# nv-tlabs/LION

Hardware: AMD Instinct MI355X
Metric: shapes/sec @1000-step DDIM, Bx2048pts (higher is better)
Workload: dtype f32 (operands of the 3x3x3 voxel convolutions and of the long 1x1 convolutions cut into fp16 hi/lo pairs on the 16-bi...

## Files before the change

### include/lion_hip.h

```cpp
#ifndef LION_HIP_H_
#define LION_HIP_H_

#include <stddef.h>
#include <stdint.h>

#ifdef __cplusplus
extern "C" {
#endif

typedef void *lionStream_t;

#define LION_OK 0
#define LION_EINVAL (-1)
#define LION_EUNSUPPORTED (-2)
#define LION_EWORKSPACE (-3)

int lion_abi_version(void);

size_t lion_avg_voxelize_workspace_bytes(int B, int C, int N, int r);
int lion_avg_voxelize_forward(const float *feat, const int32_t *coords, int B, int C, int N,
                              int r, float *out, int32_t *ind, int32_t *cnt, void *ws,
                              size_t ws_bytes, lionStream_t stream);

int lion_voxelize_points_forward(const float *feat, const float *coords, int B, int C, int N,
// ... 133 lines not shown
int lion_conv3d_stat_tiles(int r, int Cout, int B, int sparse);
int lion_conv3d_k3_fused_forward(const float *x, const float *wp, const float *bias, int B, int Cin,
                                 int Cout, int r, const float *pro_a, const float *pro_b, const float *pro_bias,
                                 const float *tconst, float *y, float *stats, int32_t *occ, lionStream_t stream);
size_t lion_conv3d_occupancy_ints(int r, int Cout, int B);
int lion_conv3d_const_response(const float *wsum, const float *bias2, const float *bias1, const float *pro_a,
                               const float *pro_b, int B, int Cin, int Cout, float *tconst, lionStream_t stream);
int lion_conv3d_tile_occupancy(const int32_t *cnt, int B, int r, int Cout, int32_t *occ_m1, int32_t *occ_m2,
                               lionStream_t stream);
int lion_conv3d_tile_occupancy_aware(const int32_t *cnt, int B, int r, int Cout, int32_t *occ_m1, int32_t *occ_m2,
                                     int consumer_aware, lionStream_t stream);
int lion_groupnorm_fold(const float *stats, int B, int C, int T, int G, int voxels, const float *gamma,
                        const float *beta, const float *fac, const float *gbias, int ld_fg, float eps,
                        float *A, float *Bs, float *chmean, lionStream_t stream);
size_t lion_conv3d_split_packed_halfs(int Cout, int Cin);
int lion_conv3d_split_pack_weights(const float *w, int Cout, int Cin, uint16_t *wp, lionStream_t stream);
int lion_conv3d_split_stat_tiles(int r, int Cout);
int lion_conv3d_k3_split_forward(const float *x, const uint16_t *wp, const float *bias, int B, int Cin, int Cout,
                                 int r, const float *pro_a, const float *pro_b, const float *pro_bias,
                                 const float *tconst, float *y, float *stats, int32_t *occ, lionStream_t stream);
int lion_conv3d_k3_half_forward(const float *x, const uint16_t *wp, const float *bias, int B, int Cin, int Cout,
                                int r, const float *pro_a, const float *pro_b, const float *pro_bias,
                                const float *tconst, float *y, float *stats, int32_t *occ, lionStream_t stream);
size_t lion_skinny_packed_floats(int Cout, int Cin);
int lion_skinny_pack_weights(const float *w, int Cout, int Cin, float *wp, lionStream_t stream);
int lion_skinny_splits(int Cin, int Cout);
int lion_skinny_gemm(const float *pin, int ks_in, const float *bias_in, int act_in, const float *addT,
                     const float *wp, int nb, int Cin, int Cout, float *pout, lionStream_t stream);
int lion_skinny_finish(const float *A, int ks_a, const float *bias_a, const float *Bp, int ks_b, const float *resid,
                       int nb, int C, int mode, float *y, lionStream_t stream);
int lion_skinny_gemm_se_finish(const float *pin, int ks_in, const float *bias_in, int act_in, const float *wp, int nb, int Cin,
                               int Cout, const float *A, int ks_a, const float *bias_a, const float *resid, float *y,
                               lionStream_t stream);
int lion_to_channel_major(const float *a, int lda, int Ca, float *oa, const float *b, int ldb, int Cb, float *ob, int B,
                          lionStream_t stream);
int lion_from_channel_major(const float *x, int B, int C, float *y, lionStream_t stream);
int lion_groupnorm_fold_se(const float *stats, int B, int C, int T, int G, int voxels, const float *gamma,
                           const float *beta, const float *fac, const float *gbias, int ld_fg, float eps, const float *w1,
                           const float *w2, int H, float *A, float *Bs, lionStream_t stream);
int lion_se_gate(const float *chmean, const float *w1, const float *w2, int B, int C, int H, float *A,
                 float *Bs, lionStream_t stream);
int lion_trilinear_devoxelize_affine_forward(const float *coords, const float *feat, const float *scale,
                                             const float *shift, int B, int C, int N, int r, float *out,
                                             lionStream_t stream);
size_t lion_devoxelize_plan_bytes(int B, int N, int r);
int lion_trilinear_devoxelize_plan(const float *coords, int B, int N, int r, void *plan, size_t plan_bytes,
                                   lionStream_t stream);
int lion_trilinear_devoxelize_planned_forward(const void *plan, size_t plan_bytes, const float *coords, const float *feat,
                                              const float *scale, const float *shift, int B, int C, int N, int r,
                                              float *out, lionStream_t stream);

int lion_row_stats(const float *x, int rows, int L, float *stats, lionStream_t stream);
size_t lion_pwconv_packed_floats(int Cout, int Cin);
int lion_pwconv_pack_weights(const float *w, int Cout, int Cin, float *wp, lionStream_t stream);
int lion_pwconv_stat_tiles(int Cout, int Cin, int L);
int lion_pwconv_forward(const float *x, const float *wp, const float *bias, int B, int Cin, int Cout, int L,
                        const float *pro_a, const float *pro_b, float *y, float *stats, lionStream_t stream);
int lion_pwconv_forward_max(const float *x, const float *wp, const float *bias, int B, int Cin, int Cout, int L,
                            const float *pro_a, const float *pro_b, const float *out_a, const float *out_b,
                            float *stats, float *ymax, lionStream_t stream);
size_t lion_pwconv_split_packed_halfs(int Cout, int Cin);
int lion_pwconv_split_pack_weights(const float *w, int Cout, int Cin, uint16_t *wp, lionStream_t stream);
int lion_pwconv_split_pack_weights_t(const float *w, int Cout, int Cin, const uint16_t *wp, uint16_t *wpt, lionStream_t stream);
int lion_pwconv_split_stat_tiles(int Cout, int Cin, int L);
int lion_pwconv_split_forward(const float *x, const uint16_t *wp, const float *bias, int B, int Cin, int Cout, int L,
                              const float *pro_a, const float *pro_b, float *y, float *stats, lionStream_t stream);
int lion_pwconv_grouped_forward(const float *coords, const float *centers, const float *feat, const int32_t *idx,
                                const float *wp, const float *bias, int B, int C, int N, int M, int U, int Cout, float *y,
                                float *stats, lionStream_t stream);
int lion_pwconv_split_grouped_forward(const float *coords, const float *centers, const float *feat, const int32_t *idx,
                                      const uint16_t *wp, const float *bias, int B, int C, int N, int M, int U, int Cout,
                                      float *y, float *stats, lionStream_t stream);
int lion_internal_pwconv_walk(const float *x, const float *wp, const float *bias, int B, int Cin, int Cout, int L,
                              const float *pro_a, const float *pro_b, const float *out_a, const float *out_b,
                              const float *coords, const float *centers, const float *feat, const int32_t *idx, int N, int U,
                              float *y, float *stats, int max_wg, int lds_weights, lionStream_t stream);
int lion_linear_attention_core(const float *qkv, int B, int H, int D, int N, float *out, lionStream_t stream);
int lion_linear_attention_core_backward(const float *qkv, const float *gout, int B, int H, int D, int N, float *gqkv,
                                        lionStream_t stream);
int lion_linear_forward(const float *x, const float *wp, const float *bias, int B, int K, int O, int act, float slope,
                        float *y, lionStream_t stream);
int lion_affine_swish(const float *x, const float *A, const float *Bs, int rows, int L, float *y,
                      lionStream_t stream);
int lion_affine_swish_max(const float *x, const float *A, const float *Bs, int rows, int M, int U,
                          float *y, lionStream_t stream);
int lion_timestep_embedding(const float *t, const float *row, float scale, int B, int half, int D, float *emb,
                            lionStream_t stream);
int lion_affine_swish_add(const float *x, const float *A, const float *Bs, const float *addend, int rows, int L, float *y,
                          lionStream_t stream);

size_t lion_scatter_csr_workspace_bytes(int B, int E, int bins);
int lion_scatter_csr(const float *gy, const int32_t *idx, const float *w, int B, int C, int S, int E, int bins, void *ws,
                     size_t ws_bytes, float *gx, lionStream_t stream);

size_t lion_pwconv_wgrad_workspace_bytes(int B, int Cin, int Cout, int L);
int lion_pwconv_wgrad(const float *x, const float *gy, int B, int Cin, int Cout, int L, void *ws, size_t ws_bytes,
                      float *gw, float *gb, lionStream_t stream);

int lion_gn_train_fold(const float *stats, const float *gw, const float *gb, const float *fac, int fac_stride,
                       const float *bias, int bias_stride, int B, int C, int G, int L, float eps, float *A, float *Bs,
                       float *mean, float *rstd, lionStream_t stream);
int lion_row_stats64(const float *x, int rows, int L, double *stats, lionStream_t stream);
int lion_gn_train_fold64(const double *stats, const float *gw, const float *gb, const float *fac, int fac_stride,
                         const float *bias, int bias_stride, int B, int C, int G, int L, float eps, float *A,
                         float *Bs, float *mean, float *rstd, lionStream_t stream);
int lion_gn_train_bwd_fold(const float *S, const float *mean, const float *rstd, const float *gw, const float *gb,
                           const float *fac, int fac_stride, int B, int C, int G, int L, float *Q, float *R, float *dfac,
                           float *dbias, int d_stride, float *pw, const float *A, const double *xstats, const float *gate,
                           const float *qse, float *Aout, lionStream_t stream);
int lion_gn_train_param_grads(const float *pw, int B, int C, float *dgw, float *dgb, float *dxs, lionStream_t stream);
// ... 71 lines not shown
```

### lion_amd/_lib.py

```python
from __future__ import annotations

import ctypes as C
import os

_HERE = os.path.dirname(os.path.abspath(__file__))
SO_PATH = os.environ.get("LION_HIP_SO") or os.path.join(_HERE, "csrc", "liblion_hip.so")

_vp, _i, _f, _sz = C.c_void_p, C.c_int, C.c_float, C.c_size_t

SIGNATURES = {
    "lion_abi_version": (_i, []),
    "lion_avg_voxelize_workspace_bytes": (_sz, [_i, _i, _i, _i]),
    "lion_avg_voxelize_forward": (_i, [_vp, _vp, _i, _i, _i, _i, _vp, _vp, _vp, _vp, _sz, _vp]),
    "lion_voxelize_points_forward": (_i, [_vp, _vp, _i, _i, _i, _i, _i, _f, _vp, _vp, _vp, _vp,
                                          _vp, _sz, _vp]),
    "lion_voxel_plan_bytes": (_sz, [_i, _i, _i]),
    "lion_voxel_index": (_i, [_vp, _i, _i, _i, _i, _f, _vp, _vp, _vp, _vp, _sz, _vp]),
    "lion_voxel_scatter": (_i, [_vp, _vp, _sz, _i, _i, _i, _i, _vp, _vp]),
    "lion_voxel_scatter_read": (_i, [_vp, _vp, _sz, _i, _i, _i, _i, _vp, _vp, _vp]),
    "lion_avg_voxelize_backward": (_i, [_vp, _vp, _vp, _i, _i, _i, _i, _vp, _vp]),
    "lion_trilinear_devoxelize_forward": (_i, [_vp, _vp, _i, _i, _i, _i, _i, _vp, _vp, _vp, _vp]),
    "lion_trilinear_devoxelize_backward": (_i, [_vp, _vp, _vp, _i, _i, _i, _i, _vp, _vp]),
    "lion_ball_query": (_i, [_vp, _vp, _i, _i, _i, _f, _i, _vp, _vp]),
    "lion_grouping_forward": (_i, [_vp, _vp, _i, _i, _i, _i, _i, _vp, _vp]),
# ... 9 lines not shown
    "lion_chamfer_loss_reduce": (_i, [_vp, _vp, _i, _i, _i, _f, _f, _vp, _vp]),
    "lion_chamfer_loss_backward": (_i, [_vp, _vp, _vp, _vp, _vp, _i, _i, _i, _f, _f, _vp, _vp, _vp]),
    "lion_emd_workspace_bytes": (_sz, [_i, _i, _i]),
    "lion_emd_approxmatch": (_i, [_vp, _vp, _i, _i, _i, _vp, _vp, _sz, _vp]),
    "lion_emd_cost": (_i, [_vp, _vp, _i, _i, _i, _vp, _vp, _sz, _vp]),
    "lion_emd_matchcost": (_i, [_vp, _vp, _vp, _i, _i, _i, _vp, _vp, _sz, _vp]),
    "lion_emd_matchcost_backward": (_i, [_vp, _vp, _vp, _vp, _i, _i, _i, _vp, _vp, _vp]),
    "lion_conv3d_packed_floats": (_sz, [_i, _i]),
    "lion_conv3d_pack_weights": (_i, [_vp, _i, _i, _vp, _vp]),
    "lion_conv3d_k3_forward": (_i, [_vp, _vp, _vp, _i, _i, _i, _i, _vp, _vp]),
    "lion_conv3d_wgrad_workspace_floats": (_sz, [_i, _i, _i, _i]),
    "lion_conv3d_k3_wgrad": (_i, [_vp, _vp, _i, _i, _i, _i, _vp, _vp, _sz, _vp]),
    "lion_conv3d_k3_wgrad_split": (_i, [_vp, _vp, _i, _i, _i, _i, _vp, _vp, _sz, _vp]),
    "lion_conv3d_wgrad_sparse_workspace_floats": (_sz, [_i, _i, _i, _i]),
    "lion_conv3d_k3_wgrad_split_sparse": (_i, [_vp, _vp, _vp, _i, _i, _i, _i, _vp, _vp, _sz, _vp]),
    "lion_conv3d_stat_tiles": (_i, [_i, _i, _i, _i]),
    "lion_conv3d_k3_fused_forward": (_i, [_vp, _vp, _vp, _i, _i, _i, _i, _vp, _vp, _vp, _vp, _vp, _vp, _vp, _vp]),
    "lion_conv3d_const_response": (_i, [_vp, _vp, _vp, _vp, _vp, _i, _i, _i, _vp, _vp]),
    "lion_conv3d_occupancy_ints": (_sz, [_i, _i, _i]),
    "lion_conv3d_tile_occupancy": (_i, [_vp, _i, _i, _i, _vp, _vp, _vp]),
    "lion_conv3d_tile_occupancy_aware": (_i, [_vp, _i, _i, _i, _vp, _vp, _i, _vp]),
    "lion_conv3d_split_packed_halfs": (_sz, [_i, _i]),
    "lion_conv3d_split_pack_weights": (_i, [_vp, _i, _i, _vp, _vp]),
    "lion_conv3d_split_stat_tiles": (_i, [_i, _i]),
    "lion_conv3d_k3_split_forward": (_i, [_vp, _vp, _vp, _i, _i, _i, _i, _vp, _vp, _vp, _vp, _vp, _vp, _vp, _vp]),
    "lion_conv3d_k3_half_forward": (_i, [_vp, _vp, _vp, _i, _i, _i, _i, _vp, _vp, _vp, _vp, _vp, _vp, _vp, _vp]),
    "lion_groupnorm_fold": (_i, [_vp, _i, _i, _i, _i, _i, _vp, _vp, _vp, _vp, _i, _f, _vp, _vp, _vp, _vp]),
    "lion_groupnorm_fold_se": (_i, [_vp, _i, _i, _i, _i, _i, _vp, _vp, _vp, _vp, _i, _f, _vp, _vp, _i, _vp, _vp, _vp]),
    "lion_skinny_packed_floats": (_sz, [_i, _i]),
    "lion_skinny_pack_weights": (_i, [_vp, _i, _i, _vp, _vp]),
    "lion_skinny_splits": (_i, [_i, _i]),
    "lion_skinny_gemm": (_i, [_vp, _i, _vp, _i, _vp, _vp, _i, _i, _i, _vp, _vp]),
    "lion_skinny_gemm_se_finish": (_i, [_vp, _i, _vp, _i, _vp, _i, _i, _i, _vp, _i, _vp, _vp, _vp, _vp]),
    "lion_skinny_finish": (_i, [_vp, _i, _vp, _vp, _i, _vp, _i, _i, _i, _vp, _vp]),
    "lion_to_channel_major": (_i, [_vp, _i, _i, _vp, _vp, _i, _i, _vp, _i, _vp]),
    "lion_from_channel_major": (_i, [_vp, _i, _i, _vp, _vp]),
    "lion_se_gate": (_i, [_vp, _vp, _vp, _i, _i, _i, _vp, _vp, _vp]),
    "lion_trilinear_devoxelize_affine_forward": (_i, [_vp, _vp, _vp, _vp, _i, _i, _i, _i, _vp, _vp]),
    "lion_devoxelize_plan_bytes": (_sz, [_i, _i, _i]),
    "lion_trilinear_devoxelize_plan": (_i, [_vp, _i, _i, _i, _vp, _sz, _vp]),
    "lion_trilinear_devoxelize_planned_forward": (_i, [_vp, _sz, _vp, _vp, _vp, _vp, _i, _i, _i, _i, _vp, _vp]),
    "lion_row_stats": (_i, [_vp, _i, _i, _vp, _vp]),
    "lion_pwconv_packed_floats": (_sz, [_i, _i]),
    "lion_pwconv_pack_weights": (_i, [_vp, _i, _i, _vp, _vp]),
    "lion_pwconv_stat_tiles": (_i, [_i, _i, _i]),
    "lion_pwconv_forward": (_i, [_vp, _vp, _vp, _i, _i, _i, _i, _vp, _vp, _vp, _vp, _vp]),
    "lion_pwconv_forward_max": (_i, [_vp, _vp, _vp, _i, _i, _i, _i, _vp, _vp, _vp, _vp, _vp, _vp, _vp]),
    "lion_pwconv_split_packed_halfs": (_sz, [_i, _i]),
    "lion_pwconv_split_pack_weights": (_i, [_vp, _i, _i, _vp, _vp]),
    "lion_pwconv_split_pack_weights_t": (_i, [_vp, _i, _i, _vp, _vp, _vp]),
    "lion_pwconv_split_stat_tiles": (_i, [_i, _i, _i]),
    "lion_pwconv_split_forward": (_i, [_vp, _vp, _vp, _i, _i, _i, _i, _vp, _vp, _vp, _vp, _vp]),
    "lion_pwconv_grouped_forward": (_i, [_vp, _vp, _vp, _vp, _vp, _vp, _i, _i, _i, _i, _i, _i, _vp, _vp, _vp]),
    "lion_pwconv_split_grouped_forward": (_i, [_vp, _vp, _vp, _vp, _vp, _vp, _i, _i, _i, _i, _i, _i, _vp, _vp, _vp]),
    "lion_internal_pwconv_walk": (_i, [_vp, _vp, _vp, _i, _i, _i, _i, _vp, _vp, _vp, _vp, _vp, _vp, _vp, _vp, _i, _i, _vp, _vp, _i, _i, _vp]),
    "lion_linear_attention_core": (_i, [_vp, _i, _i, _i, _i, _vp, _vp]),
    "lion_linear_attention_core_backward": (_i, [_vp, _vp, _i, _i, _i, _i, _vp, _vp]),
    "lion_linear_forward": (_i, [_vp, _vp, _vp, _i, _i, _i, _i, _f, _vp, _vp]),
    "lion_affine_swish": (_i, [_vp, _vp, _vp, _i, _i, _vp, _vp]),
    "lion_affine_swish_max": (_i, [_vp, _vp, _vp, _i, _i, _i, _vp, _vp]),
    "lion_timestep_embedding": (_i, [_vp, _vp, _f, _i, _i, _i, _vp, _vp]),
    "lion_affine_swish_add": (_i, [_vp, _vp, _vp, _vp, _i, _i, _vp, _vp]),
    "lion_scatter_csr_workspace_bytes": (_sz, [_i, _i, _i]),
    "lion_scatter_csr": (_i, [_vp, _vp, _vp, _i, _i, _i, _i, _i, _vp, _sz, _vp, _vp]),
    "lion_pwconv_wgrad_workspace_bytes": (_sz, [_i, _i, _i, _i]),
    "lion_pwconv_wgrad": (_i, [_vp, _vp, _i, _i, _i, _i, _vp, _sz, _vp, _vp, _vp]),
    "lion_gn_train_fold": (_i, [_vp, _vp, _vp, _vp, _i, _vp, _i, _i, _i, _i, _i, _f, _vp, _vp, _vp, _vp, _vp]),
    "lion_row_stats64": (_i, [_vp, _i, _i, _vp, _vp]),
    "lion_gn_train_fold64": (_i, [_vp, _vp, _vp, _vp, _i, _vp, _i, _i, _i, _i, _i, _f, _vp, _vp, _vp, _vp, _vp]),
    "lion_gn_train_bwd_fold": (_i, [_vp, _vp, _vp, _vp, _vp, _vp, _i, _i, _i, _i, _i, _vp, _vp, _vp, _vp, _i, _vp, _vp, _vp, _vp, _vp,
                                    _vp, _vp]),
    "lion_gn_train_param_grads": (_i, [_vp, _i, _i, _vp, _vp, _vp, _vp]),
    "lion_adam_chunk": (_i, []),
    "lion_adam_row": (_i, []),
    "lion_adam_step": (_i, [_vp, _vp, _vp, _i, _i, _vp, _f, _f, _f, _f, _f, _vp]),
    "lion_grad_sqnorm_partials": (_i, [_vp, _vp, _vp, _i, _vp, _vp]),
    "lion_grad_clip_coef": (_i, [_vp, _i, _f, _vp, _vp]),
    "lion_adam_step_scaled": (_i, [_vp, _vp, _vp, _i, _i, _vp, _f, _f, _f, _f, _f, _vp, _vp]),
    "lion_se_gate_fwd": (_i, [_vp, _vp, _vp, _i, _i, _i, _i, _vp, _vp, _vp, _vp, _vp]),
    "lion_se_gate_bwd": (_i, [_vp, _vp, _vp, _vp, _vp, _vp, _i, _i, _i, _i, _vp, _vp, _vp, _vp, _vp, _vp]),
    "lion_rows_dot2": (_i, [_vp, _vp, _vp, _i, _i, _i, _vp, _vp]),
    "lion_trilinear_devoxelize_backward_affine": (_i, [_vp, _vp, _vp, _vp, _vp, _vp, _vp, _i, _i, _i, _i, _vp, _vp]),
    "lion_gn_se_gate_fwd": (_i, [_vp, _vp, _vp, _vp, _vp, _i, _i, _i, _i, _vp, _vp, _vp, _vp, _vp, _vp]),
    "lion_gn_se_gate_bwd": (_i, [_vp, _vp, _vp, _vp, _vp, _vp, _vp, _vp, _vp, _i, _i, _i, _i, _vp, _vp, _vp, _vp, _vp, _vp, _vp]),
    "lion_affine_act": (_i, [_vp, _vp, _vp, _i, _i, _i, _vp, _vp]),
    "lion_affine_act_bwd_stats": (_i, [_vp, _vp, _vp, _vp, _i, _i, _i, _vp, _vp]),
    "lion_affine_act_bwd_apply": (_i, [_vp, _vp, _vp, _vp, _vp, _vp, _i, _i, _i, _vp, _vp]),
    "lion_affine_act_dropout": (_i, [_vp, _vp, _vp, _i, _i, _i, _vp, _f, _vp, _vp]),
    "lion_affine_act_dropout_bwd_stats": (_i, [_vp, _vp, _vp, _vp, _i, _i, _i, _vp, _f, _vp, _vp]),
# ... 107 lines not shown
```

### lion_amd/csrc/attention.hip

```cpp
#include "common.h"
#include <math.h>

namespace {

typedef float f32x16 __attribute__((ext_vector_type(16)));
constexpr int AD = 32;
constexpr int AT = 64;

__global__ __launch_bounds__(256) void linattn_core_kernel(const float *__restrict__ qkv, int H, int N,
                                                           float *__restrict__ out) {
  __shared__ float pT[AT * 33], vT[AT * 33];
  __shared__ float part[4][1024];
  __shared__ float rmax[AD], rinv[AD];
  const int tid = threadIdx.x, lane = tid & 63, wave = tid >> 6, cl = lane & 31, kh = lane >> 5;
  const int h = blockIdx.x, b = blockIdx.y;
  const size_t bs = (size_t)b * 3 * H * AD * N;
  const float *q = qkv + bs + (size_t)(0 * H + h) * AD * N;
  const float *k = qkv + bs + (size_t)(1 * H + h) * AD * N;
  const float *v = qkv + bs + (size_t)(2 * H + h) * AD * N;

  {
    const int d = tid >> 3, sub = tid & 7;
    const float *kr = k + (size_t)d * N;
    float m = -INFINITY;
// ... 31 lines not shown
    }
    __syncthreads();
  }
#pragma unroll
  for (int i = 0; i < 16; ++i) part[wave][((i & 3) + 8 * (i >> 2) + 4 * kh) * 32 + cl] = acc[i];
  __syncthreads();
  float *ctx = pT;
#pragma unroll
  for (int e = tid; e < 1024; e += 256)
    ctx[(e >> 5) * 33 + (e & 31)] = ((part[0][e] + part[1][e]) + part[2][e]) + part[3][e];
  __syncthreads();

  float av[16];
#pragma unroll
  for (int s = 0; s < 16; ++s) av[s] = ctx[(2 * s + kh) * 33 + cl];
  float *ob = out + ((size_t)b * H + h) * AD * N;
  for (int c0 = wave * 32; c0 < N; c0 += 128) {
    const int n = c0 + cl;
    const bool ok = n < N;
    const int nc = ok ? n : N - 1;
    float bv[16];
#pragma unroll
    for (int s = 0; s < 16; ++s) bv[s] = q[(size_t)(2 * s + kh) * N + nc];
    f32x16 o;
#pragma unroll
    for (int i = 0; i < 16; ++i) o[i] = 0.f;
#pragma unroll
    for (int s = 0; s < 16; ++s) o = __builtin_amdgcn_mfma_f32_32x32x2f32(av[s], ok ? bv[s] : 0.f, o, 0, 0, 0);
    if (ok) {
#pragma unroll
      for (int i = 0; i < 16; ++i) ob[(size_t)((i & 3) + 8 * (i >> 2) + 4 * kh) * N + n] = o[i];
    }
  }
}

__global__ __launch_bounds__(256) void linattn_core_bwd_kernel(const float *__restrict__ qkv, const float *__restrict__ gout,
                                                               int H, int N, float *__restrict__ gqkv) {
  __shared__ float pT[AT * 33], vT[AT * 33], qT[AT * 33], gT[AT * 33];
  __shared__ float part[4][1024];
  __shared__ float ctxs[AD * 33], gctxs[AD * 33];
  __shared__ float rmax[AD], rinv[AD], dots[AD];
  const int tid = threadIdx.x, lane = tid & 63, wave = tid >> 6, cl = lane & 31, kh = lane >> 5;
  const int h = blockIdx.x, b = blockIdx.y;
  const size_t bs = (size_t)b * 3 * H * AD * N;
  const float *q = qkv + bs + (size_t)(0 * H + h) * AD * N;
  const float *k = qkv + bs + (size_t)(1 * H + h) * AD * N;
  const float *v = qkv + bs + (size_t)(2 * H + h) * AD * N;
  const float *g = gout + ((size_t)b * H + h) * AD * N;
  float *gq = gqkv + bs + (size_t)(0 * H + h) * AD * N;
  float *gk = gqkv + bs + (size_t)(1 * H + h) * AD * N;
  float *gv = gqkv + bs + (size_t)(2 * H + h) * AD * N;

  {
    const int d = tid >> 3, sub = tid & 7;
    const float *kr = k + (size_t)d * N;
    float m = -INFINITY;
    for (int n = sub; n < N; n += 8) { const float t = kr[n]; m = t > m ? t : m; }
    for (int s = 1; s < 8; s <<= 1) { const float o = __shfl_xor(m, s, 64); m = o > m ? o : m; }
    float sum = 0.f;
    for (int n = sub; n < N; n += 8) sum += expf(kr[n] - m);
    for (int s = 1; s < 8; s <<= 1) sum += __shfl_xor(sum, s, 64);
    if (sub == 0) { rmax[d] = m; rinv[d] = 1.0f / sum; }
  }
  __syncthreads();

  f32x16 acc, gacc;
// ... 63 lines not shown
      bg[s] = ok ? g[(size_t)r_ * N + nc] : 0.f;
      bv[s] = ok ? v[(size_t)r_ * N + nc] : 0.f;
      bp[s] = ok ? expf(k[(size_t)r_ * N + nc] - rmax[r_]) * rinv[r_] : 0.f;
    }
    f32x16 oq, op, ov;
#pragma unroll
    for (int i = 0; i < 16; ++i) oq[i] = op[i] = ov[i] = 0.f;
#pragma unroll
    for (int s = 0; s < 16; ++s) {
      oq = __builtin_amdgcn_mfma_f32_32x32x2f32(aq[s], bg[s], oq, 0, 0, 0);
      op = __builtin_amdgcn_mfma_f32_32x32x2f32(ap[s], bv[s], op, 0, 0, 0);
      ov = __builtin_amdgcn_mfma_f32_32x32x2f32(av[s], bp[s], ov, 0, 0, 0);
    }
    if (ok) {
#pragma unroll
      for (int i = 0; i < 16; ++i) {
        const int row = (i & 3) + 8 * (i >> 2) + 4 * kh;
        gq[(size_t)row * N + n] = oq[i];
        gv[(size_t)row * N + n] = ov[i];
        const float pr = expf(k[(size_t)row * N + n] - rmax[row]) * rinv[row];
        gk[(size_t)row * N + n] = pr * (op[i] - dots[row]);
      }
    }
  }
}

}

extern "C" {

int lion_linear_attention_core(const float *qkv, int B, int H, int D, int N, float *out, lionStream_t stream) {
  if (!qkv || !out || B <= 0 || H <= 0 || N <= 0) return LION_EINVAL;
  if (D != AD) return LION_EUNSUPPORTED;
  return lion_launch<linattn_core_kernel>(dim3(H, B), 256, 0, static_cast<hipStream_t>(stream), qkv, H, N, out);
}

int lion_linear_attention_core_backward(const float *qkv, const float *gout, int B, int H, int D, int N, float *gqkv,
                                        lionStream_t stream) {
  if (!qkv || !gout || !gqkv || B <= 0 || H <= 0 || N <= 0) return LION_EINVAL;
  if (D != AD) return LION_EUNSUPPORTED;
  return lion_launch<linattn_core_bwd_kernel>(dim3(H, B), 256, 0, static_cast<hipStream_t>(stream), qkv, gout, H, N,
                                              gqkv);
}

}
```

### lion_amd/csrc/skinny.hip

```cpp
#include "common.h"

namespace {

typedef float f32x16 __attribute__((ext_vector_type(16)));

typedef float v4f __attribute__((ext_vector_type(4)));
__device__ __forceinline__ float4 ld_stream(const float4 *p) {
  const v4f v = __builtin_nontemporal_load(reinterpret_cast<const v4f *>(p));
  return make_float4(v.x, v.y, v.z, v.w);
}
__device__ __forceinline__ float relu_keep_nan(float v) { return !(v <= 0.f) ? v : 0.f; }

template <bool FIN>
__global__ __launch_bounds__(1024) void skinny_gemm_kernel(const float *__restrict__ pin, int ks_in,
                                                           const float *__restrict__ bias_in, int act_in,
                                                           const float *__restrict__ addT,
                                                           const float *__restrict__ wp, int Cin, int Cout,
                                                           float *__restrict__ pout, const float *__restrict__ fa, int ks_a,
                                                           const float *__restrict__ bias_a,
                                                           const float *__restrict__ resid) {
  extern __shared__ __attribute__((aligned(16))) float smem[];
  float(*part)[1024] = reinterpret_cast<float(*)[1024]>(smem);
  const int tid = threadIdx.x, lane = tid & 63, wave = tid >> 6;
  const int o0 = blockIdx.x * 32, ks = blockIdx.y, KS = gridDim.y, nb = blockIdx.z, NB = gridDim.z;
// ... 49 lines not shown
      *reinterpret_cast<float4 *>(&part[wave][g * 256 + lane * 4]) = v;
      __builtin_amdgcn_fence(__ATOMIC_RELEASE, "wavefront");
      __builtin_amdgcn_wave_barrier();
      __builtin_amdgcn_fence(__ATOMIC_ACQUIRE, "wavefront");
#pragma unroll
      for (int e = 0; e < 4; ++e) {
        const int u = 4 * g + e;
        const float a = e == 0 ? a4[g].x : e == 1 ? a4[g].y : e == 2 ? a4[g].z : a4[g].w;
        acc = __builtin_amdgcn_mfma_f32_32x32x2f32(a, part[wave][(2 * u + kh) * 32 + cl], acc, 0, 0, 0);
      }
    }
    __builtin_amdgcn_fence(__ATOMIC_RELEASE, "wavefront");
    __builtin_amdgcn_wave_barrier();
  }
  __syncthreads();
#pragma unroll
  for (int i = 0; i < 16; ++i) part[wave][((i & 3) + 8 * (i >> 2) + 4 * kh) * 32 + cl] = acc[i];
  __syncthreads();
  float s = 0.f;
#pragma unroll
  for (int w = 0; w < 16; ++w) s += part[w][tid];
  if (FIN) {
    const size_t n = (size_t)NB * Cout * 32, i = ((size_t)nb * Cout + o0 + (tid >> 5)) * 32 + (tid & 31);
    float a = bias_a ? bias_a[o0 + (tid >> 5)] : 0.f;
    for (int q = 0; q < ks_a; ++q) a += fa[(size_t)q * n + i];
    float g = 0.f;
    g += s;
    pout[i] = resid[i] + relu_keep_nan(a) * (1.0f / (1.0f + expf(-g)));
    return;
  }
  pout[((size_t)(ks * NB + nb) * Cout + o0 + (tid >> 5)) * 32 + (tid & 31)] = s;
}

__global__ __launch_bounds__(256) void skinny_finish_kernel(const float *__restrict__ A, int ks_a,
                                                            const float *__restrict__ bias_a,
                                                            const float *__restrict__ Bp, int ks_b,
                                                            const float *__restrict__ resid, int n, int C,
                                                            int mode, float *__restrict__ y) {
  const int i = blockIdx.x * 256 + threadIdx.x;
  if (i >= n) return;
  const int c = (i >> 5) % C;
  float a = bias_a ? bias_a[c] : 0.f;
  for (int q = 0; q < ks_a; ++q) a += A[(size_t)q * n + i];
  if (mode == 1) {
    float g = 0.f;
    for (int q = 0; q < ks_b; ++q) g += Bp[(size_t)q * n + i];
    a = resid[i] + relu_keep_nan(a) * (1.0f / (1.0f + expf(-g)));
  }
  y[i] = a;
}

__global__ __launch_bounds__(256) void to_channel_major_kernel(const float *__restrict__ a, int lda, int Ca, float *__restrict__ oa,
                                                               const float *__restrict__ b, int ldb, int Cb, float *__restrict__ ob,
                                                               int B, int nb) {
  const int na = a ? nb * Ca * 32 : 0, nbb = b ? nb * Cb * 32 : 0;
  for (int i = blockIdx.x * 256 + threadIdx.x; i < na + nbb; i += gridDim.x * 256) {
    const bool second = i >= na;
    const int j = second ? i - na : i, C = second ? Cb : Ca, ld = second ? ldb : lda;
    const float *src = second ? b : a;
    const int col = j & 31, c = (j >> 5) % C, blk = j / (32 * C), row = blk * 32 + col;
    (second ? ob : oa)[j] = row < B ? src[(size_t)row * ld + c] : 0.f;
  }
}
__global__ __launch_bounds__(256) void from_channel_major_kernel(const float *__restrict__ x, int B, int C, float *__restrict__ y) {
  const int i = blockIdx.x * 256 + threadIdx.x;
  if (i >= B * C) return;
  const int row = i / C, c = i - row * C;
  y[i] = x[((size_t)(row >> 5) * C + c) * 32 + (row & 31)];
}

__global__ void skinny_pack_kernel(const float *__restrict__ w, int Cout, int Cin, int ksteps4,
                                   float *__restrict__ wp) {
  const int i = blockIdx.x * blockDim.x + threadIdx.x;
  if (i >= Cout * ksteps4 * 8) return;
  const int e = i & 3, j = (i >> 2) & 31, kh = (i >> 7) & 1, s4 = (i >> 8) % ksteps4, t = i / (256 * ksteps4);
  const int k = 2 * (4 * s4 + e) + kh;
  wp[i] = k < Cin ? w[(size_t)(t * 32 + j) * Cin + k] : 0.f;
}

}

extern "C" {

size_t lion_skinny_packed_floats(int Cout, int Cin) { return (size_t)Cout * 8 * (((Cin + 1) / 2 + 3) / 4); }

int lion_skinny_pack_weights(const float *w, int Cout, int Cin, float *wp, lionStream_t stream) {
  if (!w || !wp || Cout <= 0 || Cin <= 0) return LION_EINVAL;
  if (Cout % 32 != 0) return LION_EUNSUPPORTED;
  const int ksteps4 = ((Cin + 1) / 2 + 3) / 4, total = Cout * ksteps4 * 8;
  return lion_launch<skinny_pack_kernel>(lion_cdiv(total, 256), 256, 0, static_cast<hipStream_t>(stream), w, Cout, Cin,
                                         ksteps4, wp);
}

int lion_skinny_splits(int Cin, int Cout) {
  if (Cout <= 0 || Cout % 32 != 0 || Cin <= 0) return 0;
  const int tiles = Cout / 32, ksteps = (Cin + 1) / 2;
  int ks = 1;
  while (ks < 8 && tiles * ks * 2 <= 256 && ksteps / (ks * 2 * 16) >= 8) ks *= 2;
  return ks;
}

int lion_skinny_gemm(const float *pin, int ks_in, const float *bias_in, int act_in, const float *addT,
                     const float *wp, int nb, int Cin, int Cout, float *pout, lionStream_t stream) {
  if (!pin || !wp || !pout || nb <= 0 || Cin <= 0 || Cout <= 0 || ks_in < 1 || act_in < 0 || act_in > 1)
    return LION_EINVAL;
  if (Cout % 32 != 0) return LION_EUNSUPPORTED;
  const size_t lds = (size_t)16 * 1024 * 4;
  return lion_launch<skinny_gemm_kernel<false>>(dim3(Cout / 32, lion_skinny_splits(Cin, Cout), nb), 1024, lds,
                                                static_cast<hipStream_t>(stream), pin, ks_in, bias_in, act_in, addT, wp,
                                                Cin, Cout, pout, nullptr, 0, nullptr, nullptr);
}

int lion_skinny_gemm_se_finish(const float *pin, int ks_in, const float *bias_in, int act_in, const float *wp, int nb, int Cin,
                               int Cout, const float *A, int ks_a, const float *bias_a, const float *resid, float *y,
                               lionStream_t stream) {
  if (!pin || !wp || !A || !resid || !y || nb <= 0 || Cin <= 0 || Cout <= 0 || ks_in < 1 || ks_a < 1 || act_in < 0 || act_in > 1)
    return LION_EINVAL;
  if (Cout % 32 != 0 || lion_skinny_splits(Cin, Cout) != 1) return LION_EUNSUPPORTED;
  const size_t lds = (size_t)16 * 1024 * 4;
  return lion_launch<skinny_gemm_kernel<true>>(dim3(Cout / 32, 1, nb), 1024, lds, static_cast<hipStream_t>(stream), pin,
                                               ks_in, bias_in, act_in, nullptr, wp, Cin, Cout, y, A, ks_a, bias_a,
                                               resid);
}

int lion_skinny_finish(const float *A, int ks_a, const float *bias_a, const float *Bp, int ks_b, const float *resid,
                       int nb, int C, int mode, float *y, lionStream_t stream) {
  if (!A || !y || nb <= 0 || C <= 0 || ks_a < 1 || (mode != 0 && mode != 1)) return LION_EINVAL;
  if (mode == 1 && (!Bp || !resid || ks_b < 1)) return LION_EINVAL;
  const int n = nb * C * 32;
  return lion_launch<skinny_finish_kernel>(lion_cdiv(n, 256), 256, 0, static_cast<hipStream_t>(stream), A, ks_a, bias_a,
                                           Bp, ks_b, resid, n, C, mode, y);
}

int lion_to_channel_major(const float *a, int lda, int Ca, float *oa, const float *b, int ldb, int Cb, float *ob, int B,
                          lionStream_t stream) {
  if (B <= 0 || (!a && !b) || (a && (!oa || Ca <= 0 || lda < 0)) || (b && (!ob || Cb <= 0 || ldb < 0))) return LION_EINVAL;
  const int nb = (B + 31) / 32, total = nb * 32 * ((a ? Ca : 0) + (b ? Cb : 0));
  return lion_launch<to_channel_major_kernel>(lion_cdiv(total, 256) > 64 ? 64 : lion_cdiv(total, 256), 256, 0,
                                              static_cast<hipStream_t>(stream), a, lda, Ca, oa, b, ldb, Cb, ob, B, nb);
}

int lion_from_channel_major(const float *x, int B, int C, float *y, lionStream_t stream) {
  if (!x || !y || B <= 0 || C <= 0) return LION_EINVAL;
  return lion_launch<from_channel_major_kernel>(lion_cdiv(B * C, 256), 256, 0, static_cast<hipStream_t>(stream), x, B,
                                                C, y);
}

}
```

Before: 5.694.

## Add load-ahead variants of skinny GEMM and linear attention core kernels

Adds new kernels for the skinny GEMM (templated on the split count, with vectorized float4 input loads and weight loads issued ahead of the MFMA work) and for the linear-attention core. The attention variant either stages K rows in LDS and does the softmax there, or prefetches the next V/K tile into registers. Default entry points now dispatch to these variants, and the old kernels stay reachable through internal 'plain' entry points for comparison. The intent is to hide global-load latency behind MFMA work and avoid recomputing exponentials. The cost is more template instantiations, larger LDS use (one wave per EU for attention), and alignment and N%4 conditions that fall back to the old path.

```diff
diff --git a/include/lion_hip.h b/include/lion_hip.h
--- a/include/lion_hip.h
+++ b/include/lion_hip.h
@@ -189,6 +189,11 @@
 int lion_skinny_gemm_se_finish(const float *pin, int ks_in, const float *bias_in, int act_in, const float *wp, int nb, int Cin,
                                int Cout, const float *A, int ks_a, const float *bias_a, const float *resid, float *y,
                                lionStream_t stream);
+int lion_internal_skinny_gemm_plain(const float *pin, int ks_in, const float *bias_in, int act_in, const float *addT,
+                                    const float *wp, int nb, int Cin, int Cout, float *pout, lionStream_t stream);
+int lion_internal_skinny_gemm_se_finish_plain(const float *pin, int ks_in, const float *bias_in, int act_in, const float *wp,
+                                              int nb, int Cin, int Cout, const float *A, int ks_a, const float *bias_a,
+                                              const float *resid, float *y, lionStream_t stream);
 int lion_to_channel_major(const float *a, int lda, int Ca, float *oa, const float *b, int ldb, int Cb, float *ob, int B,
                           lionStream_t stream);
 int lion_from_channel_major(const float *x, int B, int C, float *y, lionStream_t stream);
@@ -233,6 +238,8 @@
                               const float *coords, const float *centers, const float *feat, const int32_t *idx, int N, int U,
                               float *y, float *stats, int max_wg, int lds_weights, lionStream_t stream);
 int lion_linear_attention_core(const float *qkv, int B, int H, int D, int N, float *out, lionStream_t stream);
+int lion_internal_linear_attention_path(int N, int aligned);
+int lion_internal_linear_attention_core_plain(const float *qkv, int B, int H, int D, int N, float *out, lionStream_t stream);
 int lion_linear_attention_core_backward(const float *qkv, const float *gout, int B, int H, int D, int N, float *gqkv,
                                         lionStream_t stream);
 int lion_linear_forward(const float *x, const float *wp, const float *bias, int B, int K, int O, int act, float slope,
diff --git a/lion_amd/_lib.py b/lion_amd/_lib.py
--- a/lion_amd/_lib.py
+++ b/lion_amd/_lib.py
@@ -65,6 +65,8 @@
     "lion_skinny_splits": (_i, [_i, _i]),
     "lion_skinny_gemm": (_i, [_vp, _i, _vp, _i, _vp, _vp, _i, _i, _i, _vp, _vp]),
     "lion_skinny_gemm_se_finish": (_i, [_vp, _i, _vp, _i, _vp, _i, _i, _i, _vp, _i, _vp, _vp, _vp, _vp]),
+    "lion_internal_skinny_gemm_plain": (_i, [_vp, _i, _vp, _i, _vp, _vp, _i, _i, _i, _vp, _vp]),
+    "lion_internal_skinny_gemm_se_finish_plain": (_i, [_vp, _i, _vp, _i, _vp, _i, _i, _i, _vp, _i, _vp, _vp, _vp, _vp]),
     "lion_skinny_finish": (_i, [_vp, _i, _vp, _vp, _i, _vp, _i, _i, _i, _vp, _vp]),
     "lion_to_channel_major": (_i, [_vp, _i, _i, _vp, _vp, _i, _i, _vp, _i, _vp]),
     "lion_from_channel_major": (_i, [_vp, _i, _i, _vp, _vp]),
@@ -88,6 +90,8 @@
     "lion_pwconv_split_grouped_forward": (_i, [_vp, _vp, _vp, _vp, _vp, _vp, _i, _i, _i, _i, _i, _i, _vp, _vp, _vp]),
     "lion_internal_pwconv_walk": (_i, [_vp, _vp, _vp, _i, _i, _i, _i, _vp, _vp, _vp, _vp, _vp, _vp, _vp, _vp, _i, _i, _vp, _vp, _i, _i, _vp]),
     "lion_linear_attention_core": (_i, [_vp, _i, _i, _i, _i, _vp, _vp]),
+    "lion_internal_linear_attention_path": (_i, [_i, _i]),
+    "lion_internal_linear_attention_core_plain": (_i, [_vp, _i, _i, _i, _i, _vp, _vp]),
     "lion_linear_attention_core_backward": (_i, [_vp, _vp, _i, _i, _i, _i, _vp, _vp]),
     "lion_linear_forward": (_i, [_vp, _vp, _vp, _i, _i, _i, _i, _f, _vp, _vp]),
     "lion_affine_swish": (_i, [_vp, _vp, _vp, _i, _i, _vp, _vp]),
diff --git a/lion_amd/csrc/attention.hip b/lion_amd/csrc/attention.hip
--- a/lion_amd/csrc/attention.hip
+++ b/lion_amd/csrc/attention.hip
@@ -87,6 +87,187 @@
       for (int i = 0; i < 16; ++i) ob[(size_t)((i & 3) + 8 * (i >> 2) + 4 * kh) * N + n] = o[i];
     }
   }
+}
+
+constexpr int ASP = 4;
+constexpr int ATILE = AT * 33;
+
+__host__ __device__ constexpr int linattn_region_a(bool res, int N) {
+  return res ? (AD * (N + ASP) > AD * 33 ? AD * (N + ASP) : AD * 33) : 2 * ATILE;
+}
+
+template <bool RES>
+__global__ __launch_bounds__(256) __attribute__((amdgpu_waves_per_eu(1, 1))) void linattn_core_ahead_kernel(const float *__restrict__ qkv, int H, int N,
+                                                                 float *__restrict__ out) {
+  extern __shared__ __attribute__((aligned(16))) float lds[];
+  float *ra = lds;
+  float *vT = lds + linattn_region_a(RES, N);
+  float *rmax = vT + 2 * ATILE, *rinv = rmax + AD;
+  const int tid = threadIdx.x, lane = tid & 63, wave = __builtin_amdgcn_readfirstlane(tid >> 6), cl = lane & 31, kh = lane >> 5;
+  const int h = blockIdx.x, b = blockIdx.y;
+  const size_t bs = (size_t)b * 3 * H * AD * N;
+  const float *q = qkv + bs + (size_t)(0 * H + h) * AD * N;
+  const float *k = qkv + bs + (size_t)(1 * H + h) * AD * N;
+  const float *v = qkv + bs + (size_t)(2 * H + h) * AD * N;
+  const int ES = N + ASP, nq = N >> 2;
+  const float4 zero4 = make_float4(0.f, 0.f, 0.f, 0.f);
+
+  float4 vn[2], kn[2];
+  auto stage_load = [&](int n0) {
+#pragma unroll
+    for (int j = 0; j < 2; ++j) {
+      const int idx = tid + 256 * j, d = idx >> 4, n = min(n0 + 4 * (idx & 15), N - 4);
+      vn[j] = *reinterpret_cast<const float4 *>(v + (size_t)d * N + n);
+      if (!RES) kn[j] = *reinterpret_cast<const float4 *>(k + (size_t)d * N + n);
+    }
+  };
+  stage_load(0);
+
+  if (RES) {
+    const float4 *k4 = reinterpret_cast<const float4 *>(k);
+    auto rows_load = [&](int c, float4(&t)[8]) {
+#pragma unroll
+      for (int r = 0; r < 8; ++r) t[r] = k4[(size_t)(wave * 8 + r) * nq + c];
+    };
+    auto rows_store = [&](int c, const float4(&t)[8]) {
+#pragma unroll
+      for (int r = 0; r < 8; ++r) *reinterpret_cast<float4 *>(&ra[(wave * 8 + r) * ES + 4 * c]) = t[r];
+    };
+    int c0 = 0;
+    for (; c0 + 256 <= nq; c0 += 256) {
+      float4 t0[8], t1[8], t2[8], t3[8];
+      rows_load(c0 + lane, t0);
+      rows_load(c0 + 64 + lane, t1);
+      rows_load(c0 + 128 + lane, t2);
+      rows_load(c0 + 192 + lane, t3);
+      rows_store(c0 + lane, t0);
+      rows_store(c0 + 64 + lane, t1);
+      rows_store(c0 + 128 + lane, t2);
+      rows_store(c0 + 192 + lane, t3);
+    }
+    for (; c0 < nq; c0 += 64) {
+      float4 t0[8];
+      const int c = min(c0 + lane, nq - 1);
+      rows_load(c, t0);
+      rows_store(c, t0);
+    }
+    __syncthreads();
+  }
+
+  {
+    const int d = tid >> 3, sub = tid & 7;
+    const float *kg = k + (size_t)d * N;
+    float *kl = ra + d * ES;
+    float m = -INFINITY;
+    for (int n = sub; n < N; n += 64) {
+      float t[8];
+#pragma unroll
+      for (int j = 0; j < 8; ++j) { const int nn = min(n + 8 * j, N - 1); t[j] = RES ? kl[nn] : kg[nn]; }
+#pragma unroll
+      for (int j = 0; j < 8; ++j) m = t[j] > m ? t[j] : m;
+    }
+    for (int s = 1; s < 8; s <<= 1) { const float o = __shfl_xor(m, s, 64); m = o > m ? o : m; }
+    float sum = 0.f;
+    for (int n = sub; n < N; n += 64) {
+      float t[8];
+#pragma unroll
+      for (int j = 0; j < 8; ++j) { const int nn = min(n + 8 * j, N - 1); t[j] = RES ? kl[nn] : kg[nn]; }
+#pragma unroll
+      for (int j = 0; j < 8; ++j) {
+        const int nn = n + 8 * j;
+        const float ev = expf(t[j] - m);
+        sum = nn < N ? sum + ev : sum;
+        if (RES && nn < N) kl[nn] = ev;
+      }
+    }
+    for (int s = 1; s < 8; s <<= 1) sum += __shfl_xor(sum, s, 64);
+    if (sub == 0) { rmax[d] = m; rinv[d] = 1.0f / sum; }
+  }
+  __syncthreads();
+
+  f32x16 acc;
+#pragma unroll
+  for (int i = 0; i < 16; ++i) acc[i] = 0.f;
+  const float ri = rinv[cl];
+  for (int n0 = 0, buf = 0; n0 < N; n0 += AT, buf ^= 1) {
+    float *vb = vT + buf * ATILE, *pb = ra + buf * ATILE;
+#pragma unroll
+    for (int j = 0; j < 2; ++j) {
+      const int idx = tid + 256 * j, d = idx >> 4, c = 4 * (idx & 15);
+      const bool ok = n0 + c < N;
+      const float4 vv = ok ? vn[j] : zero4;
+      vb[(c + 0) * 33 + d] = vv.x; vb[(c + 1) * 33 + d] = vv.y; vb[(c + 2) * 33 + d] = vv.z; vb[(c + 3) * 33 + d] = vv.w;
+      if (!RES) {
+        const float mx = rmax[d], rv = rinv[d];
+        pb[(c + 0) * 33 + d] = ok ? expf(kn[j].x - mx) * rv : 0.f;
+        pb[(c + 1) * 33 + d] = ok ? expf(kn[j].y - mx) * rv : 0.f;
+        pb[(c + 2) * 33 + d] = ok ? expf(kn[j].z - mx) * rv : 0.f;
+        pb[(c + 3) * 33 + d] = ok ? expf(kn[j].w - mx) * rv : 0.f;
+      }
+    }
+    stage_load(n0 + AT);
+    __syncthreads();
+    float pa[8];
+    if (RES) {
+#pragma unroll
+      for (int i = 0; i < 4; ++i) {
+        const int n = n0 + 16 * wave + 4 * i;
+        const float4 e4 = *reinterpret_cast<const float4 *>(&ra[cl * ES + min(n, N - 4)]);
+        const bool ok = n < N;
+        pa[2 * i + 0] = ok ? (kh ? e4.y : e4.x) * ri : 0.f;
+        pa[2 * i + 1] = ok ? (kh ? e4.w : e4.z) * ri : 0.f;
+      }
+    }
+#pragma unroll
+    for (int u = 0; u < 8; ++u) {
+      const int nn = 2 * (wave * 8 + u) + kh;
+      const float a = RES ? pa[u] : pb[nn * 33 + cl];
+      acc = __builtin_amdgcn_mfma_f32_32x32x2f32(a, vb[nn * 33 + cl], acc, 0, 0, 0);
+    }
+  }
+  float bv[16], bn[16];
+  auto q_load = [&](int c0, float *dst) {
+    const int nc = min(c0 + cl, N - 1);
+#pragma unroll
+    for (int s = 0; s < 16; ++s) dst[s] = q[(size_t)(2 * s + kh) * N + nc];
+  };
+  q_load(wave * 32, bv);
+  __syncthreads();
+  float(*part)[1024] = reinterpret_cast<float(*)[1024]>(vT);
+#pragma unroll
+  for (int i = 0; i < 16; ++i) part[wave][((i & 3) + 8 * (i >> 2) + 4 * kh) * 32 + cl] = acc[i];
+  __syncthreads();
+  float *ctx = ra;
+#pragma unroll
+  for (int e = tid; e < 1024; e += 256)
+    ctx[(e >> 5) * 33 + (e & 31)] = ((part[0][e] + part[1][e]) + part[2][e]) + part[3][e];
+  __syncthreads();
+
+  float av[16];
+#pragma unroll
+  for (int s = 0; s < 16; ++s) av[s] = ctx[(2 * s + kh) * 33 + cl];
+  float *ob = out + ((size_t)b * H + h) * AD * N;
+  auto q_block = [&](int c0, bool whole) {
+    const int n = c0 + cl;
+    const bool ok = whole || n < N;
+    f32x16 o;
+#pragma unroll
+    for (int i = 0; i < 16; ++i) o[i] = 0.f;
+#pragma unroll
+    for (int s = 0; s < 16; ++s) o = __builtin_amdgcn_mfma_f32_32x32x2f32(av[s], ok ? bv[s] : 0.f, o, 0, 0, 0);
+    if (ok) {
+#pragma unroll
+      for (int i = 0; i < 16; ++i) ob[(size_t)((i & 3) + 8 * (i >> 2) + 4 * kh) * N + n] = o[i];
+    }
+  };
+  int c0 = wave * 32;
+  for (; c0 + 32 <= N; c0 += 128) {
+    q_load(c0 + 128, bn);
+    q_block(c0, true);
+#pragma unroll
+    for (int s = 0; s < 16; ++s) bv[s] = bn[s];
+  }
+  if (c0 < N) q_block(c0, false);
 }
 
 __global__ __launch_bounds__(256) void linattn_core_bwd_kernel(const float *__restrict__ qkv, const float *__restrict__ gout,
@@ -216,6 +397,22 @@
 int lion_linear_attention_core(const float *qkv, int B, int H, int D, int N, float *out, lionStream_t stream) {
   if (!qkv || !out || B <= 0 || H <= 0 || N <= 0) return LION_EINVAL;
   if (D != AD) return LION_EUNSUPPORTED;
+  const bool aligned = ((reinterpret_cast<uintptr_t>(qkv) | reinterpret_cast<uintptr_t>(out)) & 15) == 0;
+  const int path = lion_internal_linear_attention_path(N, aligned ? 1 : 0);
+  const size_t lds = (size_t)(linattn_region_a(path == 1, N) + 2 * ATILE + 2 * AD) * sizeof(float);
+  if (path == 1)
+    return lion_launch<linattn_core_ahead_kernel<true>>(dim3(H, B), 256, lds, static_cast<hipStream_t>(stream), qkv, H, N, out);
+  if (path == 2)
+    return lion_launch<linattn_core_ahead_kernel<false>>(dim3(H, B), 256, lds, static_cast<hipStream_t>(stream), qkv, H, N, out);
+  return lion_launch<linattn_core_kernel>(dim3(H, B), 256, 0, static_cast<hipStream_t>(stream), qkv, H, N, out);
+}
+int lion_internal_linear_attention_path(int N, int aligned) {
+  if (N <= 0 || N % 4 != 0 || !aligned) return 0;
+  return N <= 1024 ? 1 : 2;
+}
+int lion_internal_linear_attention_core_plain(const float *qkv, int B, int H, int D, int N, float *out, lionStream_t stream) {
+  if (!qkv || !out || B <= 0 || H <= 0 || N <= 0) return LION_EINVAL;
+  if (D != AD) return LION_EUNSUPPORTED;
   return lion_launch<linattn_core_kernel>(dim3(H, B), 256, 0, static_cast<hipStream_t>(stream), qkv, H, N, out);
 }
 
diff --git a/lion_amd/csrc/skinny.hip b/lion_amd/csrc/skinny.hip
--- a/lion_amd/csrc/skinny.hip
+++ b/lion_amd/csrc/skinny.hip
@@ -105,6 +105,119 @@
   pout[((size_t)(ks * NB + nb) * Cout + o0 + (tid >> 5)) * 32 + (tid & 31)] = s;
 }
 
+template <bool FIN, int QN, int CG, bool ADD>
+__global__ __launch_bounds__(1024) void skinny_gemm_ahead_kernel(const float *__restrict__ pin, const float *__restrict__ bias_in,
+                                                                 int act_in, const float *__restrict__ addT,
+                                                                 const float *__restrict__ wp, int Cin, int Cout,
+                                                                 float *__restrict__ pout, const float *__restrict__ fa, int ks_a,
+                                                                 const float *__restrict__ bias_a,
+                                                                 const float *__restrict__ resid) {
+  extern __shared__ __attribute__((aligned(16))) float smem[];
+  float(*part)[1024] = reinterpret_cast<float(*)[1024]>(smem);
+  const int tid = threadIdx.x, lane = tid & 63, wave = __builtin_amdgcn_readfirstlane(tid >> 6);
+  const int o0 = blockIdx.x * 32, ks = blockIdx.y, KS = gridDim.y, nb = blockIdx.z, NB = gridDim.z;
+  const int cl = lane & 31, kh = lane >> 5;
+  const int ksteps = (Cin + 1) >> 1;
+  const int ksteps4 = (ksteps + 3) >> 2;
+  const float4 *wt4 = reinterpret_cast<const float4 *>(wp + (size_t)blockIdx.x * (ksteps4 * 8) * 32);
+  const size_t in_stride = (size_t)NB * Cin * 32;
+  const float *xb = pin + (size_t)nb * Cin * 32;
+  const float *ab = ADD ? addT + (size_t)nb * Cin * 32 : nullptr;
+  const int per = ((ksteps + KS * 16 - 1) / (KS * 16) + 3) & ~3;
+  const int s_lo = min(ksteps, (ks * 16 + wave) * per), s_hi = min(ksteps, s_lo + per);
+  const size_t fn = (size_t)NB * Cout * 32, fi = ((size_t)nb * Cout + o0 + (tid >> 5)) * 32 + (tid & 31);
+  float fq[4] = {0.f, 0.f, 0.f, 0.f}, fb = 0.f, fr = 0.f;
+  if (FIN) {
+    if (bias_a) fb = bias_a[o0 + (tid >> 5)];
+#pragma unroll
+    for (int q = 0; q < 4; ++q) fq[q] = fa[(size_t)min(q, ks_a - 1) * fn + fi];
+    fr = resid[fi];
+  }
+  f32x16 acc;
+#pragma unroll
+  for (int i = 0; i < 16; ++i) acc[i] = 0.f;
+  for (int r0 = 0; r0 < per; r0 += 16) {
+    const int s0 = s_lo + r0;
+    float4 a4[4];
+#pragma unroll
+    for (int gg = 0; gg < 4; gg += CG) {
+      float4 x4[CG][QN], t4[CG];
+      float bq[CG];
+#pragma unroll
+      for (int c = 0; c < CG; ++c) {
+        const int g = gg + c;
+        bq[c] = 0.f;
+        t4[c] = make_float4(0.f, 0.f, 0.f, 0.f);
+#pragma unroll
+        for (int q = 0; q < QN; ++q) x4[c][q] = make_float4(0.f, 0.f, 0.f, 0.f);
+        if (s0 + 4 * g < s_hi) {
+          const int kc = min(2 * (s0 + 4 * g) + (lane >> 3), Cin - 1);
+          const unsigned off = (unsigned)kc * 32u + (unsigned)(lane & 7) * 4u;
+          if (bias_in) bq[c] = bias_in[kc];
+          if (ADD) t4[c] = *reinterpret_cast<const float4 *>(ab + off);
+#pragma unroll
+          for (int q = 0; q < QN; ++q) x4[c][q] = *reinterpret_cast<const float4 *>(xb + q * in_stride + off);
+        }
+      }
+      if (gg == 0) {
+#pragma unroll
+        for (int g = 0; g < 4; ++g)
+          a4[g] = ld_stream(&wt4[((size_t)(min(s0 + 4 * g, ksteps4 * 4 - 4) >> 2) * 2 + kh) * 32 + cl]);
+      }
+#pragma unroll
+      for (int c = 0; c < CG; ++c) {
+        const int g = gg + c;
+        float4 v = make_float4(0.f, 0.f, 0.f, 0.f);
+        if (s0 + 4 * g < s_hi) {
+          const int k = 2 * (s0 + 4 * g) + (lane >> 3);
+          v = make_float4(bq[c], bq[c], bq[c], bq[c]);
+#pragma unroll
+          for (int q = 0; q < (QN > 4 ? QN : 4); ++q) {
+            const float4 t = q < QN ? x4[c][q < QN ? q : 0] : make_float4(0.f, 0.f, 0.f, 0.f);
+            v.x += t.x; v.y += t.y; v.z += t.z; v.w += t.w;
+          }
+          if (act_in == 1) { v.x = relu_keep_nan(v.x); v.y = relu_keep_nan(v.y); v.z = relu_keep_nan(v.z); v.w = relu_keep_nan(v.w); }
+          v.x += t4[c].x; v.y += t4[c].y; v.z += t4[c].z; v.w += t4[c].w;
+          const bool live = k < Cin && (k >> 1) < s_hi;
+          if (!live) v = make_float4(0.f, 0.f, 0.f, 0.f);
+        }
+        *reinterpret_cast<float4 *>(&part[wave][g * 256 + lane * 4]) = v;
+        __builtin_amdgcn_fence(__ATOMIC_RELEASE, "wavefront");
+        __builtin_amdgcn_wave_barrier();
+        __builtin_amdgcn_fence(__ATOMIC_ACQUIRE, "wavefront");
+#pragma unroll
+        for (int e = 0; e < 4; ++e) {
+          const int u = 4 * g + e;
+          const float a = e == 0 ? a4[g].x : e == 1 ? a4[g].y : e == 2 ? a4[g].z : a4[g].w;
+          acc = __builtin_amdgcn_mfma_f32_32x32x2f32(a, part[wave][(2 * u + kh) * 32 + cl], acc, 0, 0, 0);
+        }
+      }
+    }
+    __builtin_amdgcn_fence(__ATOMIC_RELEASE, "wavefront");
+    __builtin_amdgcn_wave_barrier();
+  }
+  float a = fb;
+  if (FIN) {
+#pragma unroll
+    for (int q = 0; q < 4; ++q) a = q < ks_a ? a + fq[q] : a;
+    for (int q = 4; q < ks_a; ++q) a += fa[(size_t)q * fn + fi];
+  }
+  __syncthreads();
+#pragma unroll
+  for (int i = 0; i < 16; ++i) part[wave][((i & 3) + 8 * (i >> 2) + 4 * kh) * 32 + cl] = acc[i];
+  __syncthreads();
+  float s = 0.f;
+#pragma unroll
+  for (int w = 0; w < 16; ++w) s += part[w][tid];
+  if (FIN) {
+    float g = 0.f;
+    g += s;
+    pout[fi] = fr + relu_keep_nan(a) * (1.0f / (1.0f + expf(-g)));
+    return;
+  }
+  pout[((size_t)(ks * NB + nb) * Cout + o0 + (tid >> 5)) * 32 + (tid & 31)] = s;
+}
+
 __global__ __launch_bounds__(256) void skinny_finish_kernel(const float *__restrict__ A, int ks_a,
                                                             const float *__restrict__ bias_a,
                                                             const float *__restrict__ Bp, int ks_b,
@@ -151,6 +264,54 @@
   wp[i] = k < Cin ? w[(size_t)(t * 32 + j) * Cin + k] : 0.f;
 }
 
+template <bool FIN>
+int skinny_launch(bool plain, dim3 grid, hipStream_t st, const float *pin, int ks_in, const float *bias_in, int act_in,
+                  const float *addT, const float *wp, int Cin, int Cout, float *pout, const float *fa, int ks_a,
+                  const float *bias_a, const float *resid) {
+  const size_t lds = (size_t)16 * 1024 * 4;
+  if (plain || ks_in > 8 || Cin > (1 << 26))
+    return lion_launch<skinny_gemm_kernel<FIN>>(grid, 1024, lds, st, pin, ks_in, bias_in, act_in, addT, wp, Cin, Cout, pout,
+                                                fa, ks_a, bias_a, resid);
+  const bool add = !FIN && addT;
+  auto go = [&](auto Q) {
+    return lion_with_flags(add, [&](auto A) {
+      constexpr bool ADD = !FIN && decltype(A)::value;
+      constexpr int QN = decltype(Q)::value, CG = QN + (ADD ? 1 : 0) <= 4 ? 4 : 2;
+      return lion_launch<skinny_gemm_ahead_kernel<FIN, QN, CG, ADD>>(grid, 1024, lds, st, pin, bias_in, act_in, addT, wp, Cin,
+                                                                    Cout, pout, fa, ks_a, bias_a, resid);
+    });
+  };
+  switch (ks_in) {
+  case 1: return go(IntC<1>{});
+  case 2: return go(IntC<2>{});
+  case 3: return go(IntC<3>{});
+  case 4: return go(IntC<4>{});
+  case 5: return go(IntC<5>{});
+  case 6: return go(IntC<6>{});
+  case 7: return go(IntC<7>{});
+  default: return go(IntC<8>{});
+  }
+}
+
+int skinny_gemm_entry(bool plain, const float *pin, int ks_in, const float *bias_in, int act_in, const float *addT,
+                      const float *wp, int nb, int Cin, int Cout, float *pout, lionStream_t stream) {
+  if (!pin || !wp || !pout || nb <= 0 || Cin <= 0 || Cout <= 0 || ks_in < 1 || act_in < 0 || act_in > 1)
+    return LION_EINVAL;
+  if (Cout % 32 != 0) return LION_EUNSUPPORTED;
+  return skinny_launch<false>(plain, dim3(Cout / 32, lion_skinny_splits(Cin, Cout), nb), static_cast<hipStream_t>(stream), pin,
+                              ks_in, bias_in, act_in, addT, wp, Cin, Cout, pout, nullptr, 0, nullptr, nullptr);
+}
+
+int skinny_se_finish_entry(bool plain, const float *pin, int ks_in, const float *bias_in, int act_in, const float *wp, int nb,
+                           int Cin, int Cout, const float *A, int ks_a, const float *bias_a, const float *resid, float *y,
+                           lionStream_t stream) {
+  if (!pin || !wp || !A || !resid || !y || nb <= 0 || Cin <= 0 || Cout <= 0 || ks_in < 1 || ks_a < 1 || act_in < 0 || act_in > 1)
+    return LION_EINVAL;
+  if (Cout % 32 != 0 || lion_skinny_splits(Cin, Cout) != 1) return LION_EUNSUPPORTED;
+  return skinny_launch<true>(plain, dim3(Cout / 32, 1, nb), static_cast<hipStream_t>(stream), pin, ks_in, bias_in, act_in,
+                             nullptr, wp, Cin, Cout, y, A, ks_a, bias_a, resid);
+}
+
 }
 
 extern "C" {
@@ -175,25 +336,22 @@
 
 int lion_skinny_gemm(const float *pin, int ks_in, const float *bias_in, int act_in, const float *addT,
                      const float *wp, int nb, int Cin, int Cout, float *pout, lionStream_t stream) {
-  if (!pin || !wp || !pout || nb <= 0 || Cin <= 0 || Cout <= 0 || ks_in < 1 || act_in < 0 || act_in > 1)
-    return LION_EINVAL;
-  if (Cout % 32 != 0) return LION_EUNSUPPORTED;
-  const size_t lds = (size_t)16 * 1024 * 4;
-  return lion_launch<skinny_gemm_kernel<false>>(dim3(Cout / 32, lion_skinny_splits(Cin, Cout), nb), 1024, lds,
-                                                static_cast<hipStream_t>(stream), pin, ks_in, bias_in, act_in, addT, wp,
-                                                Cin, Cout, pout, nullptr, 0, nullptr, nullptr);
+  return skinny_gemm_entry(false, pin, ks_in, bias_in, act_in, addT, wp, nb, Cin, Cout, pout, stream);
+}
+int lion_internal_skinny_gemm_plain(const float *pin, int ks_in, const float *bias_in, int act_in, const float *addT,
+                                    const float *wp, int nb, int Cin, int Cout, float *pout, lionStream_t stream) {
+  return skinny_gemm_entry(true, pin, ks_in, bias_in, act_in, addT, wp, nb, Cin, Cout, pout, stream);
 }
 
 int lion_skinny_gemm_se_finish(const float *pin, int ks_in, const float *bias_in, int act_in, const float *wp, int nb, int Cin,
                                int Cout, const float *A, int ks_a, const float *bias_a, const float *resid, float *y,
                                lionStream_t stream) {
-  if (!pin || !wp || !A || !resid || !y || nb <= 0 || Cin <= 0 || Cout <= 0 || ks_in < 1 || ks_a < 1 || act_in < 0 || act_in > 1)
-    return LION_EINVAL;
-  if (Cout % 32 != 0 || lion_skinny_splits(Cin, Cout) != 1) return LION_EUNSUPPORTED;
-  const size_t lds = (size_t)16 * 1024 * 4;
-  return lion_launch<skinny_gemm_kernel<true>>(dim3(Cout / 32, 1, nb), 1024, lds, static_cast<hipStream_t>(stream), pin,
-                                               ks_in, bias_in, act_in, nullptr, wp, Cin, Cout, y, A, ks_a, bias_a,
-                                               resid);
+  return skinny_se_finish_entry(false, pin, ks_in, bias_in, act_in, wp, nb, Cin, Cout, A, ks_a, bias_a, resid, y, stream);
+}
+int lion_internal_skinny_gemm_se_finish_plain(const float *pin, int ks_in, const float *bias_in, int act_in, const float *wp,
+                                              int nb, int Cin, int Cout, const float *A, int ks_a, const float *bias_a,
+                                              const float *resid, float *y, lionStream_t stream) {
+  return skinny_se_finish_entry(true, pin, ks_in, bias_in, act_in, wp, nb, Cin, Cout, A, ks_a, bias_a, resid, y, stream);
 }
 
 int lion_skinny_finish(const float *A, int ks_a, const float *bias_a, const float *Bp, int ks_b, const float *resid,
```

New measurement: 5.803, median of 6. +1.9%, better.
